# AzheeeQAQ/Game-of-life-distributed

Measured on AMD Instinct MI355X. Metric: cell-updates/sec (GCUPS) at 1/2/4/8 MI355X; % of HBM roofline, higher is better.
Workload: dtype u32 bit-sliced (1 bit/cell)

## Files before the change

game-of-life-distributed_amd/csrc/gol_kernels.hip:

```cpp
#include "gol_kernels.h"
#include "gol_bits.h"
#include "gol_layout.h"
#include "gol_flip_seam.h"
#include "gol_skew_span.h"

#include <algorithm>
#include <climits>
#include <type_traits>
#include <utility>

namespace golk {
#ifndef GOL_LOOP_PAD
#define GOL_LOOP_PAD 0
#endif
#ifndef GOL_FILL_PHASES
#define GOL_FILL_PHASES 4
#endif

template <typename F, int... I>
__device__ __forceinline__ void static_for_impl(F &&f, std::integer_sequence<int, I...>) {
    (f(std::integral_constant<int, I>()), ...);
}
template <int N, typename F>
__device__ __forceinline__ void static_for(F &&f) {
// ... 686 lines not shown
            if constexpr (op == 5) {
                nx[k] = bop<kPrNext>(st.p2[t][k], s7[k], u2[k]);
                st.b0[t][k] = n0[k];
                st.b1[t][k] = n1[k];
            }
        }
        static_for<4>([&](auto i_tag) {
            constexpr int i = decltype(i_tag)::value;
            if constexpr (j + 1 == 4 * (i * NW / 4) - i + 3) {
                __builtin_amdgcn_sched_barrier(0);
                if constexpr (i == 0) l = from_left_lane_far(xn.w[WPL - 1]);
                if constexpr (i == 1) shn.w = __builtin_amdgcn_alignbit(xn.w[WPL - 1], l, 31);
                if constexpr (i == 2) r = from_right_lane_far(xn.w[0]);
                if constexpr (i == 3) shn.e = __builtin_amdgcn_alignbit(r, xn.w[0], 1);
                __builtin_amdgcn_sched_barrier(0);
            }
        });
    });
#pragma unroll
    for (int k = 0; k < WPL; ++k) {
        st.c[t][k] = x.w[k];
        x.w[k] = nx[k];
    }
}

template <int D, int KQ, int LO, int WPL>
__device__ __forceinline__ void push_group_pr_hi(Lanes<WPL> &x0, Lanes<WPL> &x1, Lanes<WPL> &x2,
                                                 PairSt<D, WPL> &st, Shifted &sh, const Lanes<WPL> &n0,
                                                 Lanes<WPL> &xn) {
    parity_fix<1>();
    Shifted nx;
    unit_pr<D, (KQ + 0 + LO) & 1, WPL>(LO, x0, sh, st, x1, nx);
    sh = nx;
    static_for<D - LO>([&](auto t_tag) {
        constexpr int t = LO + decltype(t_tag)::value;
        parity_fix<2>();
        if constexpr (t + 1 < D) {
            unit_pr<D, (KQ + 1 + t) & 1, WPL>(t, x1, sh, st, x0, nx);
            sh = nx;
            unit_pr<D, (KQ + 0 + t + 1) & 1, WPL>(t + 1, x0, sh, st, x2, nx);
            sh = nx;
            unit_pr<D, (KQ + 2 + t) & 1, WPL>(t, x2, sh, st, x1, nx);
            sh = nx;
        } else {
            unit_pr<D, (KQ + 1 + t) & 1, WPL>(t, x1, sh, st, x2, nx);
            sh = nx;
            xn = vmov_even(n0);
            __builtin_amdgcn_sched_barrier(0);
            unit_pr<D, (KQ + 2 + t) & 1, WPL>(t, x2, sh, st, xn, nx);
            sh = nx;
        }
    });
}
template <int D, int KQ, int WPL>
__device__ __forceinline__ void push_group_pr(Lanes<WPL> &x0, Lanes<WPL> &x1, Lanes<WPL> &x2, PairSt<D, WPL> &st,
                                              Shifted &sh, const Lanes<WPL> &n0, Lanes<WPL> &xn) {
    push_group_pr_hi<D, KQ, 0, WPL>(x0, x1, x2, st, sh, n0, xn);
}

template <int D, int KQ, int WPL>
__device__ __forceinline__ void pr_enter(const uint32_t (&h0)[3][D][WPL], const uint32_t (&h1)[3][D][WPL],
                                         const uint32_t (&cc)[3][D][WPL], PairSt<D, WPL> &st) {
#pragma unroll
    for (int t = 0; t < D; ++t)
#pragma unroll
        for (int k = 0; k < WPL; ++k) {
            st.c[t][k] = cc[2][t][k];
            if (((KQ + t) & 1) == 1) {
                st.a0[t][k] = h0[1][t][k];
                st.a1[t][k] = h1[1][t][k];
                st.b0[t][k] = h0[2][t][k];
                st.b1[t][k] = h1[2][t][k];
            } else {
                pair_sum(h0[1][t][k], h1[1][t][k], h0[2][t][k], h1[2][t][k], st.p0[t][k], st.p1[t][k], st.p2[t][k]);
                st.a0[t][k] = h0[2][t][k];
                st.a1[t][k] = h1[2][t][k];
            }
// ... 82 lines not shown
        else if constexpr (WPL == 2)
            __builtin_amdgcn_raw_buffer_store_b64((__attribute__((ext_vector_type(2))) unsigned){y.w[0], y.w[1]}, brs,
                                                  off, 0, GOL_SKEW_STORE_CPOL);
        else
            __builtin_amdgcn_raw_buffer_store_b128(
                (__attribute__((ext_vector_type(4))) unsigned){y.w[0], y.w[1], y.w[2], y.w[3]}, brs, off, 0,
                GOL_SKEW_STORE_CPOL);
        uint32_t pc = 0;
#pragma unroll
        for (int k = 0; k < WPL; ++k) pc += __builtin_popcount(y.w[k]);
        cnt += (ok && oi >= clo && oi < chi) ? pc : 0u;
    };
    auto hook = [&](int s, int k, const Lanes<WPL> &x) {
        if (s % SP::STEP != 0 || s == 0 || s / SP::STEP > SP::NPH) return;
        const int j = s / SP::STEP - 1;
        const int m = k - 2 * SP::P(j);
        const int row = (unsigned)m < (unsigned)SP::NROWS(j) ? SP::BASE(j) + m : SP::NEXP;
        put_lanes<WPL>(exp_mine + row * ROW, x.w);
    };

    uint32_t h0[3][D][WPL], h1[3][D][WPL], cc[3][D][WPL];
#pragma unroll
    for (int s = 0; s < 3; ++s)
#pragma unroll
        for (int t = 0; t < D; ++t)
#pragma unroll
            for (int k = 0; k < WPL; ++k) h0[s][t][k] = h1[s][t][k] = cc[s][t][k] = 0u;

    Lanes<WPL> x0 = vmov(load_next()), x1 = vmov(load_next()), x2 = vmov(load_next());
    int k = 0;
    [[maybe_unused]] unsigned long long wt0 = 0, wmain = 0, nmain = 0, wfill = 0, nfill = 0;
    auto fill = [&](auto a_tag) {
        constexpr int A = decltype(a_tag)::value;
        for (; A == D ? k <= 2 * D - 1 : (k + 2) / 2 <= A - 1; k += 3) {
            const Lanes<WPL> n0 = load_next(), n1 = load_next(), n2 = load_next();
            __builtin_amdgcn_sched_barrier(0);
            Lanes<WPL> y0 = x0, y1 = x1, y2 = x2;
            push_group_exp<D, A, WPL>(y0, y1, y2, h0, h1, cc, k, hook);
            if constexpr (A == D) {
                emit(y0, k - 2 * D);
                emit(y1, k + 1 - 2 * D);
                emit(y2, k + 2 - 2 * D);
            }
            __builtin_amdgcn_sched_barrier(0);
            if constexpr (GOL_SKEW_WAIT_TRACE) wt0 = __builtin_amdgcn_s_memrealtime();
            x0 = vmov(n0);
            x1 = vmov(n1);
            x2 = vmov(n2);
            if constexpr (GOL_SKEW_WAIT_TRACE) {
                asm volatile("s_waitcnt vmcnt(0)" ::: "memory");
                wfill += __builtin_amdgcn_s_memrealtime() - wt0;
                ++nfill;
            }
        }
    };
    static_for<SP::NPH>([&](auto j) { fill(std::integral_constant<int, SP::P(decltype(j)::value)>()); });
    fill(std::integral_constant<int, D>());
    if (phase_tr && lane == 0) phase_tr[0] = (unsigned long long)__builtin_amdgcn_s_memrealtime();
    asm volatile("s_waitcnt lgkmcnt(0)" ::: "memory");
    if (lane == 0) __hip_atomic_store(flag_mine, 1, __ATOMIC_RELAXED, __HIP_MEMORY_SCOPE_WORKGROUP);

    Lanes<WPL> q0, q1, q2;
#pragma unroll
    for (int i = 0; i < WPL; ++i) q0.w[i] = q1.w[i] = q2.w[i] = 0u;
    int qoi = -8;
    [[maybe_unused]] PairSt<D, WPL> st;
    [[maybe_unused]] Shifted sh = {0u, 0u};
// ... 20 lines not shown
            v.w[3] = q[3];
        }
        iroff += Ww * 4;
        return v;
    };
    [[maybe_unused]] auto istore = [&](const Lanes<WPL> &y) {
        if constexpr (WPL == 1)
            __builtin_amdgcn_raw_buffer_store_b32(y.w[0], brs, ivoff, isoff, GOL_SKEW_STORE_CPOL);
        else if constexpr (WPL == 2)
            __builtin_amdgcn_raw_buffer_store_b64((__attribute__((ext_vector_type(2))) unsigned){y.w[0], y.w[1]}, brs,
                                                  ivoff, isoff, GOL_SKEW_STORE_CPOL);
        else
            __builtin_amdgcn_raw_buffer_store_b128(
                (__attribute__((ext_vector_type(4))) unsigned){y.w[0], y.w[1], y.w[2], y.w[3]}, brs, ivoff, isoff,
                GOL_SKEW_STORE_CPOL);
        isoff += Ww * 4;
    };
    [[maybe_unused]] auto span_enter = [&]() {
        int rb = r;
        if constexpr (HALF) rb = min(__builtin_amdgcn_readlane(r, 0), __builtin_amdgcn_readlane(r, 32));
        irs = __builtin_amdgcn_make_buffer_rsrc(const_cast<uint32_t *>(a.src) + (size_t)(a.in.base + rb) * Ww, (short)0,
                                                -1, 0x00020000);
        ilofs = (col + (r - rb) * Ww) * 4;
        iroff = 0;
        isoff = (k - 3 - 2 * D) * Ww * 4;
    };
    [[maybe_unused]] auto span_leave = [&](int rows) {
        r += rows;
        if (r == wrap) r = 0;
        qoi = k - 3 - 2 * D;
    };
    for (int i = 0; i < GOL_LOOP_PAD; ++i) asm volatile("s_nop 0");
    if constexpr (PR) {
        constexpr int KSTART = skew_main_start(D);
        static_assert(KSTART % 6 == 0, "the pair main loop starts at an even push");
        {
            pr_enter<D, 0, WPL>(h0, h1, cc, st);
            sh = row_shifts<WPL>(x0);
            auto body = [&](auto in_tag) {
                constexpr bool IN = decltype(in_tag)::value;
                {
                    const Lanes<WPL> n0 = IN ? iload() : load_next(), n1 = IN ? iload() : load_next(),
                                     n2 = IN ? iload() : load_next();
                    if constexpr (IN) {
                        istore(q0);
                        istore(q1);
                        istore(q2);
                    } else {
                        emit(q0, qoi);
                        emit(q1, qoi + 1);
                        emit(q2, qoi + 2);
                    }
                    __builtin_amdgcn_sched_barrier(0);
                    Lanes<WPL> y0 = x0, y1 = x1, y2 = x2;
                    Lanes<WPL> xn;
                    push_group_pr<D, 0, WPL>(y0, y1, y2, st, sh, n0, xn);
                    q0 = y0;
                    q1 = y1;
                    q2 = y2;
                    qoi = k - 2 * D;
                    __builtin_amdgcn_sched_barrier(0);
                    x0 = xn;
                    if constexpr (HALF) x1 = vmov(n1); else x1 = vmov_even(n1);
                    x2 = vmov(n2);
                }
                {
                    const Lanes<WPL> n0 = IN ? iload() : load_next(), n1 = IN ? iload() : load_next(),
// ... 820 lines not shown
}

hipError_t launch_step_tb(const StepArgs &a, int depth, hipStream_t s, bool fill_skip, int wpl, bool paired) {
    if (paired && fill_skip) {
        const dim3 grid(tb_pair_blocks(a, wpl)), block(512);
        return dispatch_pair(
            depth, wpl,
            [&](auto kern) {
                hipLaunchKernelGGL(kern, grid, block, 0, s, a);
                return hipGetLastError();
            },
            a.alive != nullptr);
    }
    const int waves = tb_waves(a, wpl);
    const dim3 grid((waves + 3) / 4), block(256);
    return dispatch(depth, fill_skip, wpl, [&](auto kern) {
        hipLaunchKernelGGL(kern, grid, block, 0, s, a);
        return hipGetLastError();
    });
}

template <typename F>
static hipError_t dispatch_skew(int depth, int wpl, bool half, bool pr, F &&f) {
#define GOL_WCASE(D, WP) \
    if (!pr && !half && depth == D && wpl == WP) return f(gol_skew_kernel<D, WP>);
#define GOL_HCASE(D, WP) \
    if (!pr && half && depth == D && wpl == WP) return f(gol_skew_kernel<D, WP, true>);
#define GOL_RCASE(D, WP, HF) \
    if (pr && half == HF && depth == D && wpl == WP) return f(gol_skew_kernel<D, WP, HF, true>);
    GOL_WCASE(8, 2) GOL_WCASE(12, 2) GOL_WCASE(16, 2) GOL_WCASE(20, 2) GOL_WCASE(6, 4) GOL_WCASE(8, 4)
    GOL_WCASE(9, 4) GOL_WCASE(16, 1) GOL_WCASE(32, 1)
    GOL_HCASE(16, 2) GOL_HCASE(20, 2)
    GOL_RCASE(18, 2, false) GOL_RCASE(18, 2, true) GOL_RCASE(8, 4, false)
#undef GOL_WCASE
#undef GOL_HCASE
#undef GOL_RCASE
    return hipErrorInvalidValue;
}

bool skew_supported(int depth, int wpl, bool half, bool pr) {
    return dispatch_skew(depth, wpl, half, pr, [](auto) { return hipSuccess; }) == hipSuccess;
}

int skew_blocks_per_cu(int depth, int wpl, bool half, bool pr) {
    int b = 0;
    hipError_t e = dispatch_skew(depth, wpl, half, pr, [&](auto kern) {
        return hipOccupancyMaxActiveBlocksPerMultiprocessor(&b, kern, 512, 0);
    });
    return e == hipSuccess ? b : 0;
}

hipError_t launch_skew(const SkewArgs &p, int depth, int wpl, hipStream_t s) {
    const int tcols = (p.tiles_x + p.tx - 1) / p.tx;
    return dispatch_skew(depth, wpl, p.half != 0, p.pairs != 0, [&](auto kern) {
        hipLaunchKernelGGL(kern, dim3(tcols * p.nst), dim3(512), 0, s, p);
        return hipGetLastError();
    });
}

int tb_blocks_per_cu(int depth, int wpl) {
    int b = 0;
    hipError_t e = dispatch(depth, true, wpl, [&](auto kern) {
        return hipOccupancyMaxActiveBlocksPerMultiprocessor(&b, kern, 256, 0);
    });
    return (e == hipSuccess && b > 0) ? b : 1;
}
// ... 1104 lines not shown
```

game-of-life-distributed_amd/csrc/gol_skew_span.h:

```cpp
#pragma once

#if defined(__HIPCC__) || defined(__HIP__)
#define GOL_SPAN_FN __host__ __device__ __forceinline__
#else
#define GOL_SPAN_FN inline
#endif

namespace golk {

constexpr int skew_phase_step(int D) { return D > 20 ? 6 : 3; }
constexpr int skew_main_start(int D) { return 3 * ((2 * D + 2) / 3); }
constexpr int skew_main_end(int S, int D, bool self) { return S + (self ? 2 * D : 2 * skew_phase_step(D)); }

struct SkewBand {
    int ab, eb;
    bool bottom;
};
GOL_SPAN_FN SkewBand skew_band(int L, int nst, int stack, int sy, int pos, const int *wgt, int hcap, int D, bool pair) {
    const int A0 = (int)((long long)stack * L / nst) - D, E0 = (int)((long long)(stack + 1) * L / nst) - D;
    const long long Ls = (long long)(E0 - A0) + hcap;
    int cum = 0, tot = 0;
    for (int q = 0; q < sy; ++q) {
        tot += wgt[q];
        cum += q < pos ? wgt[q] : 0;
    }
    const int G = pair ? 6 : 3;
    SkewBand b;
    b.bottom = pos == sy - 1;
    b.ab = A0 + (int)(Ls * cum / tot) / G * G;
    b.eb = b.bottom ? E0 : A0 + (int)(Ls * (cum + wgt[pos]) / tot) / G * G;
    return b;
}

constexpr bool skew_interior_instance(int D, int wpl, bool half, bool pair) { return pair && wpl == 2 && !half && D == 18; }

struct SkewSpan {
    int k_lo, k_hi;
};

struct SkewSpanIn {
    int ab, eb;
    int D;
    bool self;
    bool pair;
    int off, wrap, rmax;
    bool half;
    int dr;
    int Ww;
    bool counts;
    bool enabled;
};

namespace span_detail {

struct Rows {
    unsigned c;
    long long cl;
    unsigned wrap;
    int lim;
};

GOL_SPAN_FN long long first_row(const Rows &h, int k) {
    return h.wrap ? (long long)((h.c + (unsigned)k) % h.wrap) : h.cl + k;
}

GOL_SPAN_FN int skip_to_good(const Rows &h, int k, int B) {
    const long long r = first_row(h, k);
    if (r <= h.lim) return 0;
    if (!h.wrap || h.lim < 0) return -1;
    return (int)(((long long)h.wrap - r + B - 1) / B) * B;
}

GOL_SPAN_FN int run_bodies(const Rows &h, int k, int B, int cap) {
    const long long n = ((long long)h.lim - first_row(h, k)) / B + 1;
    return n < cap ? (int)n : cap;
}

}

GOL_SPAN_FN SkewSpan skew_interior_span(const SkewSpanIn &in) {
    using namespace span_detail;
    const int B = in.pair ? 6 : 3;
    const int S = in.eb - in.ab, D = in.D;
    const int k0 = skew_main_start(D);
    SkewSpan none = {k0, k0};
    if (!in.enabled || in.counts || S <= 0 || S > 0x7FFFFFFF - 4 * D - 64) return none;
    if (in.half) {
        const long long apart = in.wrap > 0 && in.wrap > in.dr ? in.wrap : in.dr;
        if (in.dr < 0 || apart * in.Ww * 4 >= 0x7FFFFFFFll - 64) return none;
    }
    const int kmain = skew_main_end(S, D, in.self);
    int lo = 2 * D + 3, hi = S + 2 * D + 4 - B;
    if (hi > kmain) hi = kmain;
    if (lo < k0) lo = k0;
    const int K0 = k0 + (lo - k0 + B - 1) / B * B;
    if (hi <= K0) return none;
    const int K1 = K0 + (hi - K0 + B - 1) / B * B;
    const int nh = in.half ? 2 : 1;
    Rows h[2];
    for (int i = 0; i < nh; ++i) {
        const long long c = (long long)in.ab + (i ? in.dr : 0) + in.off + 3;
        h[i].wrap = in.wrap > 0 ? (unsigned)in.wrap : 0u;
        h[i].cl = c;
        h[i].c = 0;
        if (in.wrap > 0) {
            const long long m = c % in.wrap;
            h[i].c = (unsigned)(m < 0 ? m + in.wrap : m);
        }
        const long long top = in.wrap > 0 && in.wrap < (long long)in.rmax + 1 ? in.wrap : (long long)in.rmax + 1;
        const long long lim = top - B;
        h[i].lim = lim < -1 ? -1 : (int)lim;
    }
    SkewSpan best = none;
    int k = K0;
    for (int run = 0; run < 8 && k < K1; ++run) {
        bool found = false;
        for (int step = 0; step < 8 && k < K1; ++step) {
            int skip = 0;
            for (int i = 0; i < nh; ++i) {
                const int s = skip_to_good(h[i], k, B);
                if (s < 0) return best;
                if (s > skip) skip = s;
            }
            if (skip == 0) {
                found = true;
                break;
            }
// ... 14 lines not shown
```

game-of-life-distributed_amd/csrc/golhip_impl.h:

```cpp
#pragma once
#include <hip/hip_runtime.h>
#include <rccl/rccl.h>

#include <algorithm>
#include <atomic>
#include <chrono>
#include <condition_variable>
#include <cstdint>
#include <cstring>
#include <memory>
#include <mutex>
#include <string>
#include <vector>

#include "../../include/golhip.h"
#include "gol_kernels.h"
#include "gol_rule.h"

#define GOLHIP_HIDDEN __attribute__((visibility("hidden")))

namespace gh GOLHIP_HIDDEN {

using golk::kHalo;

int fail(int code, const char *fmt, ...) __attribute__((format(printf, 2, 3)));

constexpr int kDepths[] = {32, 24, 20, 18, 16, 12, 9, 8, 6, 4, 2, 1};
constexpr int kNumDepths = sizeof(kDepths) / sizeof(kDepths[0]);
constexpr int64_t kTraceWords = 8 + 2 * 1024 * 64;

template <typename T>
struct DevScratch {
    T *p = nullptr;
    int64_t cap = 0;
    int ensure(golhip *h, int64_t n, bool zero = false, int64_t floor = 1);
    hipError_t release() {
        const hipError_t e = hipFree(p);
        if (e == hipSuccess) {
            p = nullptr;
            cap = 0;
        }
        return e;
    }
};

struct Counters {
    int64_t step_launches = 0, step_turns = 0;
    int64_t skew_launches = 0, skew_half_launches = 0, pair_launches = 0, pair_turns = 0;
    int64_t persist_launches = 0, persist_turns = 0, lds_launches = 0;
    int64_t halo_exchanges = 0, halo_bytes = 0;
    int64_t flip_launches = 0, flip_entries = 0;
    int64_t flip_resident = 0;
    int64_t view_frames = 0;
    int64_t pad_launches = 0;
    int64_t rule_launches = 0;
};
struct Millis {
    double step = 0, persist = 0, flip = 0, halo = 0, view = 0;
};

struct CkptDrain {
// ... 25 lines not shown

struct golhip {
    int W = 0, H = 0, Ww = 0;
    int row0 = 0, rows = 0;
    bool strip = false;
    int device = 0;
    uint32_t flags = 0;
    hipStream_t stream = nullptr;
    bool own_stream = false;

    uint32_t *buf[2] = {nullptr, nullptr};
    int cur = 0;
    int64_t phys_rows = 0;

    int tb_depth = 20;
    int rows_per_wave = 0;
    int cu_count = 0;
    int dev_cu = 0;
    int fill_skip = 1;
    uint32_t birth = 0x008, survive = 0x00C;
    int rule_kernel = 0;
    bool conway() const { return birth == 0x008 && survive == 0x00C; }
    bool rule_path() const { return !conway() || rule_kernel != 0; }
    int last_variant = 1;
    int skew = 1;
    int skew_young = 0;
    int skew_hcap = -1;
    int skew_prio = 0;
    int skew_tx = 0;
    int skew_half = 0;
    int lds_bpc[4] = {};
    int64_t lds_bpc_bytes[4] = {};
    int lds_bpc_stride[4] = {};
    int skew_bpc[gh::kNumDepths][12] = {};
    int skew_pairs = 5;
    int skew_interior = 1;
    unsigned *skew_err = nullptr;
    unsigned *skew_err_dev = nullptr;
    int lds_band = -1;
    int lds_depth = 0;
    int lds_xcd = 1;
    int lds_waves = 0;
    int lds_wg_cu = 1;
    int lds_stride = 1;
    int resident_fault = 0;
    int lds_age = 0;
    int lds_pre = 2;
    gh::DevScratch<uint32_t> lds_edge;
    int persistent = -1;
    int wpl_opt = 0;
    bool no_quads = false;
    int persist_depth = 0;
    int persist_waves = 0;
    int paired_bands = 1;
    int dummy_rows = 0;
    int persist_wg_tx = 0;
    int persist_half = 1;
    unsigned long long *d_trace = nullptr;
    unsigned *d_sync = nullptr;
    unsigned *h_err = nullptr;
    bool persist_pending = false;
    gh::DevScratch<uint32_t> backup;
    bool guarded = false;
    bool guard_light = false;
    bool err_clear = true;
    int resident_max = (int)golk::kResidentMaxTurns;
    int64_t persist_fallbacks = 0;
    int64_t persist_timeout_ticks = 100000000ll;
    int auto_rpw[gh::kNumDepths] = {};
    bool loaded = false;
    int il = 0;
    std::atomic<int64_t> turns{0};

    unsigned long long *d_scalars = nullptr;
    unsigned long long *h_scalars = nullptr;
    int64_t alive_turn = -1;
    gh::DevScratch<unsigned long long> d_blk;
    gh::DevScratch<int32_t> d_xy;
    gh::DevScratch<unsigned long long> d_run;
    gh::DevScratch<unsigned long long> d_ftstatus;
    gh::DevScratch<unsigned> d_ftticket;
    gh::DevScratch<unsigned> d_ftctl;
    gh::DevScratch<unsigned char> d_ev;
    unsigned flip_epoch = 0;
    int flip_debug = 0;
    int flip_cp_groups = 4;
    int flip_overlap = 2;
    gh::DevScratch<unsigned> d_ftdone;
    bool ft_ticket = false;
    uint64_t ft_est = 0;
    int64_t flip_fallbacks = 0;
    gh::DevScratch<unsigned long long> d_goff;
    void *g_stage = nullptr;
    size_t g_stage_bytes = 0;
    uint64_t group_ft_est = 0;
    gh::DevScratch<uint8_t> d_stage;
    gh::DevScratch<uint32_t> d_vcount;
    bool flips_valid = false;
    int64_t flips_turn = -1;
    bool flips_counted = false;

    ncclComm_t comm = nullptr;
// ... 44 lines not shown
    if (cap >= n) return GOLHIP_OK;
    if (p) HIP_OR_FAIL(hipFree(p));
    p = nullptr;
    cap = 0;
    const int64_t want = std::max(n, floor);
    if (hipError_t e = hipMalloc((void **)&p, (size_t)want * sizeof(T)); e != hipSuccess) {
        p = nullptr;
        return fail(GOLHIP_EHIP, "hipMalloc(%lld x %zu bytes): %s", (long long)want, sizeof(T), hipGetErrorString(e));
    }
    if (zero) HIP_OR_FAIL(hipMemsetAsync(p, 0, (size_t)want * sizeof(T), h->stream));
    cap = want;
    return GOLHIP_OK;
}

int check(golhip_t h);
int set_dev(golhip_t h);
void *mapped_device_ptr(const void *p, size_t bytes, int *device = nullptr);
int span_begin(golhip_t h, hipStream_t st);
int span_end(golhip_t h, int kind, bool drain = false);
int drain_events(golhip_t h);
int take_skew_err(golhip_t h);
int sync_stream(golhip_t h);
int set_layout(golhip_t h, int il);
int loaded_canonical(golhip_t h);

struct DepthRun {
    int d;
    int64_t n;
};
struct HaloRun {
    int d, k;
};
int largest_depth(int64_t want);
DepthRun depth_plan(int cap, int64_t left);
int sched_rows(golhip_t h);
int persist_nw_for(golhip_t h, int depth, int wpl);
bool persist_on(golhip_t h);
int wpl_for(golhip_t h);
int want_il(golhip_t h);
int depth_cap(golhip_t h, bool halo);
int next_depth(golhip_t h, int64_t remaining, bool halo);
bool tb_paired(golhip_t h);
int rows_per_wave_for(golhip_t h, int depth);
void halo_plan(int strip_rows, int nranks, int rank, int depth, int Ww, golhip_halo_plan_t *p);
bool skew_dims(golhip_t h, int depth, int wpl, int L, golk::SkewArgs *sk);
bool skew_plan(golhip_t h, int depth, int wpl, const golk::StepArgs &a, golk::SkewArgs *sk);
int halo_launches(int rows, int depth, int64_t run);
HaloRun halo_next(int cap, int rows, bool resident, int64_t left);
bool lds_fits(golhip_t h, int wpl, golk::LdsBandArgs *out = nullptr);
int persist_depth_for(golhip_t h, int wpl);

golk::StepArgs step_args(golhip_t h, unsigned long long *alive, bool halo);
int exchange_rccl(golhip_t h, int depth, hipStream_t st);
int launch_depth(golhip_t h, int depth, bool count, bool halo);
int step_checked_locked(golhip_t h, int64_t nturns, int32_t want_flips);
int group_check(golhip_t *hs, int32_t n, bool need_board = true);
int group_step_locked(golhip_t *hs, int32_t n, int64_t nturns, int32_t want_flips, hipEvent_t *keep = nullptr,
                      bool pad = true);
int group_rounds(golhip_t *ss, golhip_t *owners, int32_t n, int64_t turns, bool count_last, hipEvent_t *ready);
int group_exchange(golhip_t *hs, int32_t n, int x, hipEvent_t *ready, bool relaunch = true);

int start_flips(golhip_t h);

struct ShadowPart {
    int device = 0;
    int64_t row0 = 0, rows = 0;
    uint32_t *shadow = nullptr;
// ... 34 lines not shown
```

game-of-life-distributed_amd/csrc/golhip_plan.cpp:

```cpp
#include "golhip_impl.h"
#include "gol_skew_span.h"
#include <climits>
#include <functional>

namespace gh GOLHIP_HIDDEN {

int largest_depth(int64_t want) {
    for (int d : kDepths)
        if (d <= want && d != 9 && d != 18) return d;
    return 1;
}
static bool special_depth(int d) { return d == 9 || d == 18; }

DepthRun depth_plan(int cap, int64_t left) {
    const int M = special_depth(cap) ? cap : largest_depth(std::max(1, cap));
    if (left <= 0) return {M, 0};
    const int64_t head = std::max<int64_t>(0, left / M - 12);
    const int t = (int)(left - head * M);
    std::vector<int> nl(t + 1, INT_MAX), mn(t + 1, 0), pick(t + 1, 0);
    nl[0] = 0;
    mn[0] = INT_MAX;
    for (int v = 1; v <= t; ++v)
        for (int d : kDepths) {
            if (d > M || d > v || nl[v - d] == INT_MAX || (special_depth(d) && M != d)) continue;
            const int n = nl[v - d] + 1, m = std::min(mn[v - d], d);
            if (n < nl[v] || (n == nl[v] && m > mn[v])) {
                nl[v] = n;
                mn[v] = m;
                pick[v] = d;
            }
        }
    std::vector<int> seq;
    for (int v = t; v > 0; v -= pick[v]) seq.push_back(pick[v]);
    std::sort(seq.begin(), seq.end(), std::greater<int>());
    const int d = head > 0 ? M : seq[0];
    int64_t n = head;
    for (int x : seq) n += (x == d);
    return {d, n};
}

int sched_rows(golhip_t h) { return (h->ringed() && h->nranks > 1 && h->ring_rows > 0) ? h->ring_rows : h->rows; }

static double slots_per_word(int wpl) { return 9.0 + 8.0 / wpl; }

static double plan_rate(golhip_t h, int wpl, int nw, int depth) {
    const int tiles = golk::tb_tiles(h->Ww, wpl);
    const double util = (double)h->Ww / (tiles * 62.0 * wpl);
    const double S = (double)sched_rows(h) * tiles / std::max(1.0, (double)h->cu_count * nw);
    const double occ = nw >= 16 ? 1.0 : 0.95;
    return util * S / (S + 1.75 * depth) * occ / slots_per_word(wpl);
}

static int default_depth(golhip_t h, int wpl) { return largest_depth(std::min(h->tb_depth, golk::persist_max_depth(wpl))); }

int persist_nw_for(golhip_t h, int depth, int wpl) {
    if (h->persist_waves > 0) return h->persist_waves;
    const int def = golk::persist_waves_for(depth, wpl);
    if (def == 16 && plan_rate(h, wpl, 8, depth) > plan_rate(h, wpl, 16, depth) &&
        golk::persist_blocks_per_cu(depth, wpl, 8) >= 1)
        return 8;
    return def;
}

static constexpr int64_t kPersistAutoMaxBytes = 64ll << 20;
static int wpl_per_launch(golhip_t h);
static bool skew_fills(golhip_t h);
bool persist_on(golhip_t h) {
    if (h->rule_path()) return false;
    if (h->ringed() && h->nranks > 1) return false;
    if (h->persistent >= 0) return h->persistent != 0;
    if (h->skew && skew_fills(h)) return false;
// ... 36 lines not shown
        int cap = std::min(h->tb_depth, golk::kRuleMaxDepth);
        if (halo) cap = std::min(cap, sched_rows(h));
        return cap == 9 ? 8 : cap;
    }
    const int wpl = wpl_for(h);
    int cap = std::min(h->tb_depth, (halo && persist_on(h)) ? golk::persist_max_depth(wpl) : golk::max_depth_for(wpl));
    if (halo) cap = std::min(cap, sched_rows(h));
    bool pair = false;
    if ((h->skew_pairs & 1) && wpl == 2 && cap >= 18) {
        golk::SkewArgs sk{};
        if (skew_dims(h, 18, 2, halo ? sched_rows(h) : h->rows, &sk) && (!sk.half || (h->skew_pairs & 4))) {
            cap = 18;
            pair = true;
        }
    }
    if (!pair && !halo && wpl == 2 && cap > 16) {
        golk::SkewArgs sk{};
        if (skew_dims(h, 20, 2, h->rows, &sk) && sk.half) cap = 16;
    }
    if (cap == 9 && (wpl != 4 || (halo && persist_on(h)))) cap = 8;
    if (cap == 18 && !pair) cap = 16;
    if ((h->skew_pairs & 2) && wpl == 4 && cap >= 8) {
        golk::SkewArgs sk{};
        if (skew_dims(h, 8, 4, halo ? sched_rows(h) : h->rows, &sk) && !sk.half) cap = 8;
    }
    return cap;
}

int next_depth(golhip_t h, int64_t remaining, bool halo) { return depth_plan(depth_cap(h, halo), remaining).d; }

static int depth_index(int d) {
    for (int i = 0; i < kNumDepths; ++i)
        if (kDepths[i] == d) return i;
    return kNumDepths - 1;
}

bool tb_paired(golhip_t h) { return h->paired_bands && h->fill_skip; }

int rows_per_wave_for(golhip_t h, int depth) {
    if (h->rows_per_wave > 0) return h->rows_per_wave;
    int &c = h->auto_rpw[depth_index(depth)];
    if (c == 0 && h->rule_path()) {
        const int slots =
            h->cu_count * golk::rule_wave_slots_per_cu(depth, h->W, h->birth, h->survive, h->rule_kernel == 2);
        c = golk::auto_rows_per_wave(h->Ww, h->rows, depth, std::max(slots, 1), false, 1, false);
    }
    if (c == 0) {
        const int wpl = wpl_for(h);
        const int slots = h->cu_count * golk::tb_wave_slots_per_cu(depth, wpl, tb_paired(h));
        c = golk::auto_rows_per_wave(h->Ww, h->rows, depth, std::max(slots, 1), h->fill_skip, wpl, tb_paired(h));
    }
    return c;
}

void halo_plan(int strip_rows, int nranks, int rank, int depth, int Ww, golhip_halo_plan_t *p) {
    p->prev_rank = (rank - 1 + nranks) % nranks;
    p->next_rank = (rank + 1) % nranks;
    p->rows = depth;
    p->send_up_row = kHalo;
    p->recv_bottom_row = kHalo + strip_rows;
    p->send_down_row = kHalo + strip_rows - depth;
    p->recv_top_row = kHalo - depth;
    p->bytes = (int64_t)depth * Ww * 4;
}

static int skew_bpc(golhip_t h, int depth, int wpl, bool half, bool pr) {
    int &c = h->skew_bpc[depth_index(depth)][(wpl == 4 ? 2 : wpl - 1) + (half ? 3 : 0) + (pr ? 6 : 0)];
    if (c == 0) {
        const int b = golk::skew_blocks_per_cu(depth, wpl, half, pr);
        c = b > 0 ? b : -1;
    }
    return c;
}

bool skew_dims(golhip_t h, int depth, int wpl, int L, golk::SkewArgs *sk) {
    const bool pr = (depth == 18 && (h->skew_pairs & 1)) || (wpl == 4 && depth == 8 && (h->skew_pairs & 2));
    if (!h->skew || h->W % 32 != 0 || !golk::skew_supported(depth, wpl, false, pr)) return false;
    const int hcap = h->skew_hcap >= 0 ? h->skew_hcap : 3 * depth / 4;
    const int smin = depth + 3;
    const bool half_ok = h->skew_half >= 0 && L % 2 == 0 && golk::skew_supported(depth, wpl, true, pr);
    int best_tx = 0, best_nst = 0, best_half = 0, best_tiles = 0;
    double best = 1e300;
    for (int half = 0; half <= (half_ok ? 1 : 0); ++half) {
        if (!half && half_ok && h->skew_half > 0) continue;
        const int bpc = skew_bpc(h, depth, wpl, half, pr);
        if (bpc < 1) continue;
        const int tiles = half ? (h->Ww + golk::kHalfTileValid * wpl - 1) / (golk::kHalfTileValid * wpl)
                               : golk::tb_tiles(h->Ww, wpl);
        const int Lh = half ? L / 2 : L;
        for (int tx = 1; tx <= 2; ++tx) {
            if (h->skew_tx && tx != h->skew_tx) continue;
            const int sy = 8 / tx, tcols = (tiles + tx - 1) / tx;
            const int nst = std::min(h->cu_count * bpc / tcols,
                                     Lh / (sy * (smin + hcap) - hcap));
            if (nst < 1) continue;
            if (h->skew == 1 && (int64_t)nst * tcols * 4 < (int64_t)h->cu_count * bpc * 3) continue;
            if (((double)Lh / nst + hcap + (half ? Lh : 0)) * h->Ww * 4 >= 2147483648.0) continue;
            const double per_wave = ((double)Lh / nst + hcap) / sy * (half ? 1.02 : 1.0);
            if (per_wave < best * 0.999) {
                best = per_wave;
                best_tx = tx;
                best_nst = nst;
                best_half = half;
                best_tiles = tiles;
            }
        }
    }
    if (!best_tx) return false;
    sk->tiles_x = best_tiles;
    sk->pairs = pr ? 1 : 0;
    sk->interior = h->skew_interior && golk::skew_interior_instance(depth, wpl, best_half != 0, pr);
    sk->tx = best_tx;
    sk->nst = best_nst;
    sk->half = best_half;
    sk->hcap = hcap;
    return true;
}

static bool skew_fills(golhip_t h) {
    if (!h->skew || h->W % 32 != 0) return false;
    const int wpl = wpl_per_launch(h);
    int cap = std::min(h->tb_depth, golk::max_depth_for(wpl));
    if (cap == 9 && wpl != 4) cap = 8;
    const int depth = cap == 9 ? 9 : largest_depth(cap);
    golk::SkewArgs sk{};
    return skew_dims(h, depth, wpl, sched_rows(h), &sk);
}

bool skew_plan(golhip_t h, int depth, int wpl, const golk::StepArgs &a, golk::SkewArgs *sk) {
    if (!skew_dims(h, depth, wpl, a.rows_out, sk)) return false;
    if (!h->skew_err) {
        void *p = nullptr, *d = nullptr;
        if (hipHostMalloc(&p, sizeof(unsigned), hipHostMallocMapped) != hipSuccess) return false;
        if (hipHostGetDevicePointer(&d, p, 0) != hipSuccess) {
            (void)hipHostFree(p);
            return false;
        }
        h->skew_err = static_cast<unsigned *>(p);
        h->skew_err_dev = static_cast<unsigned *>(d);
        *h->skew_err = 0;
    }
    const int sy = 8 / sk->tx;
    const int young = h->skew_young > 0 ? h->skew_young
                      : wpl == 4             ? 78
                      : sk->half             ? 60
                      : a.in.wrap > 0        ? (sk->pairs ? 80 : 70)
                                             : 68;
    for (int q = 0; q < 8; ++q) sk->wgt[q] = (q < sy && q * sk->tx >= 4) ? young : 100;
    sk->prio_young = h->skew_prio;
    sk->error = h->skew_err_dev;
    sk->trace = h->d_trace;
// ... 53 lines not shown
        out->Ww = h->Ww;
        out->rows = h->rows;
        out->nb = nb;
        out->D = D;
        out->hmax = hmax;
        out->xcd = h->lds_xcd;
        out->nt = nt;
        out->stride = stride;
        out->rt_stride = h->lds_stride ? 0 : 1;
        out->fault = h->resident_fault != 0;
        out->pre = h->lds_pre;
        const bool whole = wpl == 2 && P2 % 64 == 0;
        out->age = h->lds_age > 0 ? h->lds_age : !whole ? 100 : waves == 16 ? 60 : 70;
    }
    return true;
}

}

using namespace gh;

extern "C" {

int golhip_halo_schedule(int32_t strip_rows, int32_t tb_depth, int32_t resident, int64_t turns_left,
                         int32_t *depth, int32_t *launches) {
    if (!depth || !launches || strip_rows <= 0 || tb_depth < 1 || tb_depth > GOLHIP_MAX_TB_DEPTH || turns_left < 1)
        return fail(GOLHIP_EINVAL, "bad halo schedule request");
    const HaloRun hr = halo_next(std::min(tb_depth, strip_rows), strip_rows, resident != 0, turns_left);
    *depth = hr.d;
    *launches = hr.k;
    return GOLHIP_OK;
}

int golhip_skew_span(const golhip_skew_span_in_t *in, int32_t *k_lo, int32_t *k_hi) {
    if (!in || !k_lo || !k_hi || in->depth < 4 || in->depth > GOLHIP_MAX_TB_DEPTH || in->eb < in->ab || in->dr < 0 || in->row_words < 1)
        return fail(GOLHIP_EINVAL, "bad skew span request");
    const golk::SkewSpan s = golk::skew_interior_span(golk::SkewSpanIn{
        in->ab, in->eb, in->depth, in->self != 0, in->pair != 0, in->off, in->wrap, in->rmax, in->half != 0, in->dr, in->row_words,
        in->counts != 0, in->enabled != 0});
    *k_lo = s.k_lo;
    *k_hi = s.k_hi;
    return GOLHIP_OK;
}

int golhip_skew_interior_plan(golhip_t h, int32_t depth, int32_t ext, int32_t counts, int64_t *interior_bodies,
                              int64_t *main_bodies) {
    if (int rc = check(h)) return rc;
    if (!interior_bodies || !main_bodies || depth < 1 || ext < 0) return fail(GOLHIP_EINVAL, "bad skew interior request");
    std::lock_guard<std::mutex> g(h->mu);
    *interior_bodies = *main_bodies = 0;
    const bool halo = h->halo_mode();
    if (ext > 0 && !halo) return fail(GOLHIP_EINVAL, "extended rows: strips only");
    golk::StepArgs a = step_args(h, nullptr, halo);
    if (ext > 0) {
        a.rows_out = h->rows + 2 * ext;
        a.in.off = kHalo - ext;
        a.count_lo = ext;
        a.count_hi = ext + h->rows;
    }
    golk::SkewArgs sk{};
    const int wpl = wpl_for(h);
    if (!skew_plan(h, depth, wpl, a, &sk)) return GOLHIP_OK;
    const int sy = 8 / sk.tx, L = sk.half ? a.rows_out / 2 : a.rows_out, B = sk.pairs ? 6 : 3;
    for (int stack = 0; stack < sk.nst; ++stack)
        for (int pos = 0; pos < sy; ++pos) {
            const golk::SkewBand b = golk::skew_band(L, sk.nst, stack, sy, pos, sk.wgt, sk.hcap, depth, sk.pairs != 0);
            const golk::SkewSpan s = golk::skew_interior_span(golk::SkewSpanIn{
                b.ab, b.eb, depth, b.bottom, sk.pairs != 0, a.in.off, a.in.wrap, a.in.rmax, sk.half != 0, L, a.Ww,
                counts != 0 && a.count_lo < a.count_hi, sk.interior != 0});
            const int k0 = golk::skew_main_start(depth), k1 = golk::skew_main_end(b.eb - b.ab, depth, b.bottom);
            *interior_bodies += (int64_t)(s.k_hi - s.k_lo) / B * sk.tiles_x;
            *main_bodies += (int64_t)(std::max(k1 - k0, 0) + B - 1) / B * sk.tiles_x;
        }
    return GOLHIP_OK;
}

int golhip_halo_plan(int32_t width, int32_t strip_rows, int32_t nranks, int32_t rank, int32_t depth,
                     golhip_halo_plan_t *out) {
    if (!out || width <= 0 || strip_rows <= 0 || nranks < 1 || rank < 0 || rank >= nranks || depth < 1 ||
        depth > GOLHIP_HALO_ROWS || depth > strip_rows)
        return fail(GOLHIP_EINVAL, "bad halo plan request");
    halo_plan(strip_rows, nranks, rank, depth, (width + 31) / 32, out);
    return GOLHIP_OK;
}

}
```

game-of-life-distributed_amd/csrc/golhip_step.cpp:

```cpp
#include "golhip_impl.h"

namespace gh GOLHIP_HIDDEN {

golk::StepArgs step_args(golhip_t h, unsigned long long *alive, bool halo) {
    golk::StepArgs a{};
    a.src = h->buf[h->cur];
    a.dst = h->buf[h->cur ^ 1];
    a.W = h->W;
    a.Ww = h->Ww;
    a.rows_out = h->rows;
    a.dst_base = kHalo;
    if (!halo) {
        a.in.base = kHalo;
        a.in.wrap = h->H;
        a.in.off = 0;
        a.in.rmax = h->H - 1;
    } else {
        a.in.base = 0;
        a.in.wrap = 0;
        a.in.off = kHalo;
        a.in.rmax = (int)h->phys_rows - 1;
    }
    a.rows_per_wave = h->rows_per_wave;
    a.dummy_rows = h->dummy_rows > 0 ? h->dummy_rows : kHalo;
// ... 308 lines not shown
    if ((h->ringed() && h->nranks > 1) || !h->guarded) return false;
    const int wpl = wpl_for(h);
    if (d != persist_depth_for(h, wpl)) return false;
    const int e = (k - 1) * d;
    golk::StepArgs a = step_args(h, nullptr, true);
    shift_rows(a, -e, h->rows + e);
    return persist_launch(h, a, k, d, wpl, count, rc);
}

static int step_locked(golhip_t h, int64_t nturns, int32_t want_flips) {
    if (int rc = set_layout(h, want_il(h))) return rc;
    h->flips_valid = false;
    int64_t left = nturns;
    const int64_t tail = want_flips ? 1 : 0;
    const bool halo = h->halo_mode();
    if (pad_wanted(h, left - tail)) {
        bool ran = false;
        if (int rc = pad_step(h, left - tail, &ran)) return rc;
        if (ran) left = tail;
    }
    if (!halo) {
        for (;;) {
            int rc = GOLHIP_OK;
            const int64_t n = try_persist(h, left - tail, tail == 0, &rc);
            if (rc) return rc;
            if (n <= 0) break;
            left -= n;
        }
    } else if (h->nranks == 1 && persist_on(h) && h->W % 32 == 0 && !h->guarded) {
        int rc = GOLHIP_OK;
        take_guard(h, &rc);
        if (rc) return rc;
    }
    while (left > tail) {
        if (!halo) {
            const int d = depth_plan(depth_cap(h, false), left - tail).d;
            if (int rc = launch_depth(h, d, left - d == 0, false)) return rc;
            left -= d;
            continue;
        }
        const HaloRun hr = halo_next(depth_cap(h, true), sched_rows(h), persist_on(h), left - tail);
        const int d = hr.d, k = hr.k;
        if (int rc = exchange_rccl(h, k * d, h->stream)) return rc;
        int prc = GOLHIP_OK;
        if (try_persist_halo(h, d, k, left - k * d == 0, &prc)) {
            left -= (int64_t)k * d;
            continue;
        }
        if (prc) return prc;
        for (int i = 0; i < k; ++i) {
            if (int rc = launch_ext(h, d, left - d == 0, (k - 1 - i) * d)) return rc;
            left -= d;
        }
    }
    if (want_flips && nturns > 0) {
        if (halo)
            if (int rc = exchange_rccl(h, 1, h->stream)) return rc;
        if (int rc = launch_depth(h, 1, true, halo)) return rc;
        if (int rc = start_flips(h)) return rc;
    }
    return GOLHIP_OK;
}

int step_checked_locked(golhip_t h, int64_t nturns, int32_t want_flips) {
    if (!h->loaded) return fail(GOLHIP_EINVAL, "no board loaded");
    if (h->nranks == 1 && !h->torus()) return fail(GOLHIP_EINVAL, "strip handle needs golhip_comm_init or golhip_group_step");
    if (int rc = set_dev(h)) return rc;
    const int64_t turns0 = h->turns;
    const int cur0 = h->cur;
// ... 263 lines not shown
```

include/golhip.h:

```cpp
#ifndef GOLHIP_H
#define GOLHIP_H

#include <stddef.h>
#include <stdint.h>

#ifdef __cplusplus
extern "C" {
#endif

#define GOLHIP_OK 0
#define GOLHIP_EINVAL (-1)
#define GOLHIP_EHIP (-2)
#define GOLHIP_ENOMEM (-3)
#define GOLHIP_ERANGE (-4)
#define GOLHIP_ERCCL (-5)
#define GOLHIP_ECORRUPT (-6)

#define GOLHIP_FLAG_TIMING 0x1u

#define GOLHIP_UNIQUE_ID_BYTES 128
#define GOLHIP_MAX_TB_DEPTH 32
#define GOLHIP_HALO_ROWS 128

typedef struct golhip golhip;
// ... 58 lines not shown
int golhip_set_rows_per_wave(golhip_t h, int32_t rows);
int golhip_set_option(golhip_t h, const char *key, int64_t value);
int golhip_set_pad_step(golhip_t h, int32_t mode);

int golhip_rule_parse(const char *text, uint32_t *birth, uint32_t *survive);
int golhip_rule_format(uint32_t birth, uint32_t survive, char *out, uint64_t cap);
int golhip_set_rule(golhip_t h, uint32_t birth, uint32_t survive);
int golhip_rule(golhip_t h, uint32_t *birth, uint32_t *survive);

int golhip_comm_unique_id(uint8_t id[GOLHIP_UNIQUE_ID_BYTES]);
int golhip_comm_init(golhip_t h, const uint8_t id[GOLHIP_UNIQUE_ID_BYTES], int32_t nranks, int32_t rank);
int golhip_comm_info(golhip_t h, int32_t *nranks, int32_t *rank, int32_t *ring_rows);

typedef int (*golhip_test_transport_fn)(void *user, int32_t prev_rank, int32_t next_rank, const void *send_up,
                                        const void *send_down, void *recv_top, void *recv_bottom, int64_t bytes);
int golhip_test_ring_init(golhip_t h, int32_t nranks, int32_t rank, int32_t ring_rows, golhip_test_transport_fn fn,
                          void *user);

int golhip_group_step(golhip_t *hs, int32_t n, int64_t nturns);
int golhip_group_step_ex(golhip_t *hs, int32_t n, int64_t nturns, int32_t want_flips);
int golhip_group_set_pad_step(golhip_t *hs, int32_t n, int32_t mode);

typedef struct golhip_halo_plan {
    int32_t prev_rank, next_rank;
    int32_t send_up_row, recv_top_row;
    int32_t send_down_row, recv_bottom_row;
    int32_t rows;
    int64_t bytes;
} golhip_halo_plan_t;
int golhip_halo_plan(int32_t width, int32_t strip_rows, int32_t nranks, int32_t rank, int32_t depth,
                     golhip_halo_plan_t *out);
int golhip_halo_schedule(int32_t strip_rows, int32_t tb_depth, int32_t resident, int64_t turns_left,
                         int32_t *depth, int32_t *launches);
typedef struct golhip_skew_span_in {
    int32_t ab, eb, depth, self, pair;
    int32_t off, wrap, rmax;
    int32_t half, dr, row_words, counts, enabled;
} golhip_skew_span_in_t;
int golhip_skew_span(const golhip_skew_span_in_t *in, int32_t *k_lo, int32_t *k_hi);
int golhip_skew_interior_plan(golhip_t h, int32_t depth, int32_t ext, int32_t counts, int64_t *interior_bodies,
                              int64_t *main_bodies);

int golhip_load_bytes(golhip_t h, const uint8_t *cells);
int golhip_load_bits(golhip_t h, const uint32_t *words);
int golhip_fill_random(golhip_t h, uint64_t seed);

int golhip_step(golhip_t h, int64_t nturns, int32_t want_flips);
int golhip_sync(golhip_t h);
int golhip_turn(golhip_t h, int64_t *turns_done);

int golhip_alive_count(golhip_t h, uint64_t *count, int64_t *at_turn);
int golhip_alive_count_global(golhip_t h, uint64_t *count, int64_t *at_turn);
int golhip_flips(golhip_t h, int32_t *xy, uint64_t cap, uint64_t *n);
int golhip_step_flips(golhip_t h, int64_t nturns, int32_t *xy, uint64_t cap, uint64_t *counts, uint64_t *n);
#define GOLHIP_FLIPS_XY 0
#define GOLHIP_FLIPS_INDEX 1
int golhip_flip_stream(golhip_t h, int64_t nturns, int32_t format, void *out, uint64_t cap, uint64_t *counts,
                       int64_t *turns_done, uint64_t *n);
int golhip_group_flip_stream(golhip_t *hs, int32_t n, int64_t nturns, int32_t format, void *out, uint64_t cap,
                             uint64_t *counts, int64_t *turns_done, uint64_t *n_entries);
int golhip_alive_cells(golhip_t h, int32_t *xy, uint64_t cap, uint64_t *n);
int golhip_snapshot_bytes(golhip_t h, uint8_t *out);
int golhip_snapshot_bits(golhip_t h, uint32_t *out);
int golhip_snapshot_rows(golhip_t h, int32_t row, int32_t nrows, uint32_t *out);
int golhip_board_hash(golhip_t h, uint64_t *hash);

// ... 96 lines not shown
```

Before: 148,800.

## Add pair-kernel tail depths and cost-based depth scheduling for remainder turns

Instantiates the paired skew kernel for depths 12, 15 and 16, adjusting the pair main-loop start to an even push, and adds a launch-cost model in depth_plan. The model picks a sequence of tail launches that minimises estimated cost using the cheaper pair kernels. This targets the tail turns that previously fell back to non-pair or smaller-depth launches. It adds more kernel instantiations (code size, compile time) and scheduling barriers, and depends on a heuristic cost model.

```diff
diff --git a/game-of-life-distributed_amd/csrc/gol_kernels.hip b/game-of-life-distributed_amd/csrc/gol_kernels.hip
--- a/game-of-life-distributed_amd/csrc/gol_kernels.hip
+++ b/game-of-life-distributed_amd/csrc/gol_kernels.hip
@@ -742,6 +742,7 @@
     Shifted nx;
     unit_pr<D, (KQ + 0 + LO) & 1, WPL>(LO, x0, sh, st, x1, nx);
     sh = nx;
+    __builtin_amdgcn_sched_barrier(0);
     static_for<D - LO>([&](auto t_tag) {
         constexpr int t = LO + decltype(t_tag)::value;
         parity_fix<2>();
@@ -753,6 +754,7 @@
             unit_pr<D, (KQ + 2 + t) & 1, WPL>(t, x2, sh, st, x1, nx);
             sh = nx;
         } else {
+            __builtin_amdgcn_sched_barrier(0);
             unit_pr<D, (KQ + 1 + t) & 1, WPL>(t, x1, sh, st, x2, nx);
             sh = nx;
             xn = vmov_even(n0);
@@ -901,7 +903,8 @@
     [[maybe_unused]] unsigned long long wt0 = 0, wmain = 0, nmain = 0, wfill = 0, nfill = 0;
     auto fill = [&](auto a_tag) {
         constexpr int A = decltype(a_tag)::value;
-        for (; A == D ? k <= 2 * D - 1 : (k + 2) / 2 <= A - 1; k += 3) {
+        constexpr int KFILL = skew_main_start(D, PR) != skew_main_start(D) ? skew_main_start(D, PR) - 1 : 2 * D - 1;
+        for (; A == D ? k <= KFILL : (k + 2) / 2 <= A - 1; k += 3) {
             const Lanes<WPL> n0 = load_next(), n1 = load_next(), n2 = load_next();
             __builtin_amdgcn_sched_barrier(0);
             Lanes<WPL> y0 = x0, y1 = x1, y2 = x2;
@@ -988,7 +991,7 @@
     };
     for (int i = 0; i < GOL_LOOP_PAD; ++i) asm volatile("s_nop 0");
     if constexpr (PR) {
-        constexpr int KSTART = skew_main_start(D);
+        constexpr int KSTART = skew_main_start(D, PR);
         static_assert(KSTART % 6 == 0, "the pair main loop starts at an even push");
         {
             pr_enter<D, 0, WPL>(h0, h1, cc, st);
@@ -1875,6 +1878,7 @@
     GOL_WCASE(9, 4) GOL_WCASE(16, 1) GOL_WCASE(32, 1)
     GOL_HCASE(16, 2) GOL_HCASE(20, 2)
     GOL_RCASE(18, 2, false) GOL_RCASE(18, 2, true) GOL_RCASE(8, 4, false)
+    GOL_RCASE(12, 2, false) GOL_RCASE(15, 2, false) GOL_RCASE(16, 2, false)
 #undef GOL_WCASE
 #undef GOL_HCASE
 #undef GOL_RCASE
diff --git a/game-of-life-distributed_amd/csrc/gol_skew_span.h b/game-of-life-distributed_amd/csrc/gol_skew_span.h
--- a/game-of-life-distributed_amd/csrc/gol_skew_span.h
+++ b/game-of-life-distributed_amd/csrc/gol_skew_span.h
@@ -10,6 +10,10 @@
 
 constexpr int skew_phase_step(int D) { return D > 20 ? 6 : 3; }
 constexpr int skew_main_start(int D) { return 3 * ((2 * D + 2) / 3); }
+constexpr int skew_main_start(int D, bool pair) {
+    return pair ? 6 * ((skew_main_start(D) + 5) / 6) : skew_main_start(D);
+}
+constexpr bool skew_pair_tail_depth(int D) { return D == 12 || D == 15 || D == 16; }
 constexpr int skew_main_end(int S, int D, bool self) { return S + (self ? 2 * D : 2 * skew_phase_step(D)); }
 
 struct SkewBand {
@@ -32,7 +36,9 @@
     return b;
 }
 
-constexpr bool skew_interior_instance(int D, int wpl, bool half, bool pair) { return pair && wpl == 2 && !half && D == 18; }
+constexpr bool skew_interior_instance(int D, int wpl, bool half, bool pair) {
+    return pair && wpl == 2 && !half && (D == 18 || skew_pair_tail_depth(D));
+}
 
 struct SkewSpan {
     int k_lo, k_hi;
@@ -82,7 +88,7 @@
     using namespace span_detail;
     const int B = in.pair ? 6 : 3;
     const int S = in.eb - in.ab, D = in.D;
-    const int k0 = skew_main_start(D);
+    const int k0 = skew_main_start(D, in.pair);
     SkewSpan none = {k0, k0};
     if (!in.enabled || in.counts || S <= 0 || S > 0x7FFFFFFF - 4 * D - 64) return none;
     if (in.half) {
@@ -92,7 +98,7 @@
     const int kmain = skew_main_end(S, D, in.self);
     int lo = 2 * D + 3, hi = S + 2 * D + 4 - B;
     if (hi > kmain) hi = kmain;
-    if (lo < k0) lo = k0;
+    if (lo < k0 + 3) lo = k0 + 3;
     const int K0 = k0 + (lo - k0 + B - 1) / B * B;
     if (hi <= K0) return none;
     const int K1 = K0 + (hi - K0 + B - 1) / B * B;
diff --git a/game-of-life-distributed_amd/csrc/golhip_impl.h b/game-of-life-distributed_amd/csrc/golhip_impl.h
--- a/game-of-life-distributed_amd/csrc/golhip_impl.h
+++ b/game-of-life-distributed_amd/csrc/golhip_impl.h
@@ -27,6 +27,7 @@
 
 constexpr int kDepths[] = {32, 24, 20, 18, 16, 12, 9, 8, 6, 4, 2, 1};
 constexpr int kNumDepths = sizeof(kDepths) / sizeof(kDepths[0]);
+constexpr int kDepthSlots = kNumDepths + 1;
 constexpr int64_t kTraceWords = 8 + 2 * 1024 * 64;
 
 template <typename T>
@@ -118,8 +119,9 @@
     int lds_bpc[4] = {};
     int64_t lds_bpc_bytes[4] = {};
     int lds_bpc_stride[4] = {};
-    int skew_bpc[gh::kNumDepths][12] = {};
+    int skew_bpc[gh::kDepthSlots][12] = {};
     int skew_pairs = 5;
+    bool pair_tail_step = false;
     int skew_interior = 1;
     unsigned *skew_err = nullptr;
     unsigned *skew_err_dev = nullptr;
@@ -153,7 +155,7 @@
     int resident_max = (int)golk::kResidentMaxTurns;
     int64_t persist_fallbacks = 0;
     int64_t persist_timeout_ticks = 100000000ll;
-    int auto_rpw[gh::kNumDepths] = {};
+    int auto_rpw[gh::kDepthSlots] = {};
     bool loaded = false;
     int il = 0;
     std::atomic<int64_t> turns{0};
@@ -264,7 +266,8 @@
     int d, k;
 };
 int largest_depth(int64_t want);
-DepthRun depth_plan(int cap, int64_t left);
+DepthRun depth_plan(int cap, int64_t left, bool pair_tail = false);
+bool pair_tail_on(golhip_t h);
 int sched_rows(golhip_t h);
 int persist_nw_for(golhip_t h, int depth, int wpl);
 bool persist_on(golhip_t h);
diff --git a/game-of-life-distributed_amd/csrc/golhip_plan.cpp b/game-of-life-distributed_amd/csrc/golhip_plan.cpp
--- a/game-of-life-distributed_amd/csrc/golhip_plan.cpp
+++ b/game-of-life-distributed_amd/csrc/golhip_plan.cpp
@@ -12,11 +12,45 @@
 }
 static bool special_depth(int d) { return d == 9 || d == 18; }
 
-DepthRun depth_plan(int cap, int64_t left) {
+static constexpr int kPairTailDepths[] = {18, 16, 15, 12, 8, 6, 4, 2, 1};
+static constexpr int kRampTenths = 281;
+static int64_t launch_cost(int d, bool pair_kernel) { return (int64_t)(10 * d + kRampTenths) * (pair_kernel ? 12 : 13); }
+static bool pair_tail_depth(int d) { return d == 18 || golk::skew_pair_tail_depth(d); }
+
+static DepthRun first_run(std::vector<int> &seq, int M, int64_t head) {
+    std::sort(seq.begin(), seq.end(), std::greater<int>());
+    const int d = head > 0 ? M : seq[0];
+    int64_t n = head;
+    for (int x : seq) n += (x == d);
+    return {d, n};
+}
+
+DepthRun depth_plan(int cap, int64_t left, bool pair_tail) {
     const int M = special_depth(cap) ? cap : largest_depth(std::max(1, cap));
     if (left <= 0) return {M, 0};
     const int64_t head = std::max<int64_t>(0, left / M - 12);
     const int t = (int)(left - head * M);
+    std::vector<int> cheap;
+    int64_t cheap_cost = -1;
+    if (pair_tail && M == 18) {
+        std::vector<int64_t> cost(t + 1, INT64_MAX);
+        std::vector<int> nl(t + 1, 0), mn(t + 1, INT_MAX), pick(t + 1, 0);
+        cost[0] = 0;
+        for (int v = 1; v <= t; ++v)
+            for (int d : kPairTailDepths) {
+                if (d > v) continue;
+                const int64_t c = cost[v - d] + launch_cost(d, pair_tail_depth(d));
+                const int n = nl[v - d] + 1, m = std::min(mn[v - d], d);
+                if (c < cost[v] || (c == cost[v] && (n < nl[v] || (n == nl[v] && m > mn[v])))) {
+                    cost[v] = c;
+                    nl[v] = n;
+                    mn[v] = m;
+                    pick[v] = d;
+                }
+            }
+        for (int v = t; v > 0; v -= pick[v]) cheap.push_back(pick[v]);
+        cheap_cost = cost[t];
+    }
     std::vector<int> nl(t + 1, INT_MAX), mn(t + 1, 0), pick(t + 1, 0);
     nl[0] = 0;
     mn[0] = INT_MAX;
@@ -32,11 +66,12 @@
         }
     std::vector<int> seq;
     for (int v = t; v > 0; v -= pick[v]) seq.push_back(pick[v]);
-    std::sort(seq.begin(), seq.end(), std::greater<int>());
-    const int d = head > 0 ? M : seq[0];
-    int64_t n = head;
-    for (int x : seq) n += (x == d);
-    return {d, n};
+    if (cheap_cost >= 0) {
+        int64_t c = 0;
+        for (int x : seq) c += launch_cost(x, pair_tail_depth(x));
+        if (cheap_cost < c) return first_run(cheap, M, head);
+    }
+    return first_run(seq, M, head);
 }
 
 int sched_rows(golhip_t h) { return (h->ringed() && h->nranks > 1 && h->ring_rows > 0) ? h->ring_rows : h->rows; }
@@ -139,7 +174,7 @@
 static int depth_index(int d) {
     for (int i = 0; i < kNumDepths; ++i)
         if (kDepths[i] == d) return i;
-    return kNumDepths - 1;
+    return d == 15 ? kNumDepths : kNumDepths - 1;
 }
 
 bool tb_paired(golhip_t h) { return h->paired_bands && h->fill_skip; }
@@ -180,8 +215,9 @@
     return c;
 }
 
-bool skew_dims(golhip_t h, int depth, int wpl, int L, golk::SkewArgs *sk) {
-    const bool pr = (depth == 18 && (h->skew_pairs & 1)) || (wpl == 4 && depth == 8 && (h->skew_pairs & 2));
+static bool skew_dims_for(golhip_t h, int depth, int wpl, int L, bool tail, golk::SkewArgs *sk) {
+    const bool pr = (depth == 18 && (h->skew_pairs & 1)) || (wpl == 4 && depth == 8 && (h->skew_pairs & 2)) ||
+                    (tail && wpl == 2 && golk::skew_pair_tail_depth(depth) && golk::skew_supported(depth, 2, false, true));
     if (!h->skew || h->W % 32 != 0 || !golk::skew_supported(depth, wpl, false, pr)) return false;
     const int hcap = h->skew_hcap >= 0 ? h->skew_hcap : 3 * depth / 4;
     const int smin = depth + 3;
@@ -224,6 +260,22 @@
     return true;
 }
 
+bool skew_dims(golhip_t h, int depth, int wpl, int L, golk::SkewArgs *sk) {
+    return skew_dims_for(h, depth, wpl, L, h->pair_tail_step, sk);
+}
+
+bool pair_tail_on(golhip_t h) {
+    if (!h->torus() || h->halo_mode() || h->rule_path() || !(h->skew_pairs & 1)) return false;
+    if (depth_cap(h, false) != 18) return false;
+    for (int d : {18, 16, 15, 12}) {
+        golk::SkewArgs sk{};
+        if (!golk::skew_supported(d, 2, false, true) || !skew_dims_for(h, d, 2, h->rows, true, &sk) || sk.half ||
+            !sk.pairs)
+            return false;
+    }
+    return true;
+}
+
 static bool skew_fills(golhip_t h) {
     if (!h->skew || h->W % 32 != 0) return false;
     const int wpl = wpl_per_launch(h);
@@ -343,6 +395,20 @@
     return GOLHIP_OK;
 }
 
+int golhip_depth_schedule(int32_t cap, int32_t pair_tail, int64_t turns_left, int32_t *depth, int64_t *launches) {
+    if (!depth || !launches || cap < 1 || cap > GOLHIP_MAX_TB_DEPTH || turns_left < 1 || (pair_tail && cap != 18))
+        return fail(GOLHIP_EINVAL, "bad depth schedule request");
+    const DepthRun run = depth_plan(cap, turns_left, pair_tail != 0);
+    *depth = run.d;
+    *launches = run.n;
+    return GOLHIP_OK;
+}
+
+int64_t golhip_launch_cost(int32_t depth, int32_t pair_kernel) {
+    if (depth < 1 || depth > GOLHIP_MAX_TB_DEPTH) return -1;
+    return launch_cost(depth, pair_kernel != 0);
+}
+
 int golhip_skew_span(const golhip_skew_span_in_t *in, int32_t *k_lo, int32_t *k_hi) {
     if (!in || !k_lo || !k_hi || in->depth < 4 || in->depth > GOLHIP_MAX_TB_DEPTH || in->eb < in->ab || in->dr < 0 || in->row_words < 1)
         return fail(GOLHIP_EINVAL, "bad skew span request");
@@ -371,7 +437,10 @@
     }
     golk::SkewArgs sk{};
     const int wpl = wpl_for(h);
-    if (!skew_plan(h, depth, wpl, a, &sk)) return GOLHIP_OK;
+    h->pair_tail_step = !halo && ext == 0 && pair_tail_on(h);
+    const bool planned = skew_plan(h, depth, wpl, a, &sk);
+    h->pair_tail_step = false;
+    if (!planned) return GOLHIP_OK;
     const int sy = 8 / sk.tx, L = sk.half ? a.rows_out / 2 : a.rows_out, B = sk.pairs ? 6 : 3;
     for (int stack = 0; stack < sk.nst; ++stack)
         for (int pos = 0; pos < sy; ++pos) {
@@ -379,7 +448,7 @@
             const golk::SkewSpan s = golk::skew_interior_span(golk::SkewSpanIn{
                 b.ab, b.eb, depth, b.bottom, sk.pairs != 0, a.in.off, a.in.wrap, a.in.rmax, sk.half != 0, L, a.Ww,
                 counts != 0 && a.count_lo < a.count_hi, sk.interior != 0});
-            const int k0 = golk::skew_main_start(depth), k1 = golk::skew_main_end(b.eb - b.ab, depth, b.bottom);
+            const int k0 = golk::skew_main_start(depth, sk.pairs != 0), k1 = golk::skew_main_end(b.eb - b.ab, depth, b.bottom);
             *interior_bodies += (int64_t)(s.k_hi - s.k_lo) / B * sk.tiles_x;
             *main_bodies += (int64_t)(std::max(k1 - k0, 0) + B - 1) / B * sk.tiles_x;
         }
diff --git a/game-of-life-distributed_amd/csrc/golhip_step.cpp b/game-of-life-distributed_amd/csrc/golhip_step.cpp
--- a/game-of-life-distributed_amd/csrc/golhip_step.cpp
+++ b/game-of-life-distributed_amd/csrc/golhip_step.cpp
@@ -364,9 +364,15 @@
         take_guard(h, &rc);
         if (rc) return rc;
     }
+    const bool pair_tail = !halo && left > tail && pair_tail_on(h);
+    struct TailFlag {
+        golhip_t h;
+        ~TailFlag() { h->pair_tail_step = false; }
+    } tail_flag{h};
+    h->pair_tail_step = pair_tail;
     while (left > tail) {
         if (!halo) {
-            const int d = depth_plan(depth_cap(h, false), left - tail).d;
+            const int d = depth_plan(depth_cap(h, false), left - tail, pair_tail).d;
             if (int rc = launch_depth(h, d, left - d == 0, false)) return rc;
             left -= d;
             continue;
diff --git a/include/golhip.h b/include/golhip.h
--- a/include/golhip.h
+++ b/include/golhip.h
@@ -114,6 +114,8 @@
                      golhip_halo_plan_t *out);
 int golhip_halo_schedule(int32_t strip_rows, int32_t tb_depth, int32_t resident, int64_t turns_left,
                          int32_t *depth, int32_t *launches);
+int golhip_depth_schedule(int32_t cap, int32_t pair_tail, int64_t turns_left, int32_t *depth, int64_t *launches);
+int64_t golhip_launch_cost(int32_t depth, int32_t pair_kernel);
 typedef struct golhip_skew_span_in {
     int32_t ab, eb, depth, self, pair;
     int32_t off, wrap, rmax;
```

Result: faster. 150,300 (median of 6 runs) (+1.0%).
